# lfilipozzi/PathPlanning

Hardware: AMD Instinct MI355X
Metric: hybrid_astar_plans_per_sec_1024x1024 (higher is better)
Workload: dtype f64

## Files before the change

### pathplanning_amd/csrc/pp_pipeline.hpp

```cpp
#pragma once

#include <chrono>
#include <cstring>
#include <deque>
#include <unordered_map>

namespace {

__global__ void __launch_bounds__(256) k_pipe_scatter(int n, const int32_t* __restrict__ slotList, const double* __restrict__ startsIn, const double* __restrict__ goalsIn,
	const uint64_t* __restrict__ seedsIn, double* __restrict__ starts, double* __restrict__ goals, uint64_t* __restrict__ seeds, MapView m, float urgentClearance, PipeCtl* ctl,
	unsigned long long* __restrict__ urgent, unsigned long long urgentMask, int* __restrict__ claimed)
{
	const int i = (int)(blockIdx.x * blockDim.x + threadIdx.x);
	bool isUrgent = false;
	uint32_t entry = 0;
	if (i < n) {
		entry = (uint32_t)slotList[i];
		const size_t s = (size_t)(entry & pph::kSlotMask);
		for (int k = 0; k < 3; k++) {
			starts[3 * s + k] = startsIn[3 * (size_t)i + k];
			goals[3 * s + k] = goalsIn[3 * (size_t)i + k];
		}
		seeds[s] = seedsIn[i];
		if (claimed) {
// ... 248 lines not shown
{
	pp_planner* pl = P->pl;
	PP_HIP_TRY(pipe_stage_ctl(P, &P->ctl->nSubmitted, P->nSubmitted));
	PP_HIP_TRY(hipEventRecord(P->evCtl, P->ctlStream));
	hipStream_t s = nullptr;
	for (int i = 0; i < kPipeSearchStreams && !s; i++) {
		const int k = (P->nextSearch + i) % kPipeSearchStreams;
		if (hipStreamQuery(P->searchStream[k]) == hipSuccess) {
			s = P->searchStream[k];
			P->nextSearch = (k + 1) % kPipeSearchStreams;
		}
	}
	if (!s) {
		P->lastLaunch = std::chrono::steady_clock::now();
		return PP_OK;
	}
	PP_HIP_TRY(hipStreamWaitEvent(s, P->evCtl, 0));
	pl->args.rowsWaves = P->waves;
	pl->args.m = pl->map->view();
	const pp_pipeline::Timed tm = timed_take(P, s, 1, 0);
	PP_HIP_TRY(pipe_dispatch_search(P, s, pl->args));
	timed_done(P, s, tm);
	P->lastLaunch = std::chrono::steady_clock::now();
	return PP_OK;
}

bool pipe_dead(const pp_pipeline* P)
{
	if (P->dead)
		set_error("the pipeline failed earlier and must be destroyed");
	return P->dead;
}
int pipe_check(const pp_pipeline* P)
{
	if (!P) {
		set_error("null pipeline");
		return PP_ERR_INVALID;
	}
	return pipe_dead(P) ? PP_ERR_HIP : PP_OK;
}


int pipe_resolve(const pp_pipeline* P, int n, const uint64_t* tickets, const char* verb, bool distinct, std::vector<int32_t>& slots)
{
	pph::TicketTable::Resolved r = P->tickets.resolve(n, tickets, verb, distinct);
	slots.swap(r.slots);
	if (r.error.empty())
		return PP_OK;
	set_error(r.error);
	return PP_ERR_INVALID;
}
int pipe_refuse(const pp_pipeline* P, uint64_t ticket, const char* verb)
{
	std::vector<int32_t> none;
	if (pipe_resolve(P, 1, &ticket, verb, false, none) == PP_OK)
		set_error("ticket " + std::to_string(ticket) + " is not a completed, held query");
	return PP_ERR_INVALID;
}

bool pipe_release(pp_pipeline* P, uint64_t ticket)
{
	P->postIndexOfTicket.erase(ticket);
	return P->tickets.release(ticket);
}

hipError_t pipe_grow(pp_pipeline* P, size_t& capacity, size_t wanted, std::initializer_list<std::pair<pph::DeviceMem*, size_t>> buffers)
{
	const bool idle = P->nSubmitted == P->doneHead;
	if (idle)
		P->heldParked.clear();
	if (capacity >= wanted)
		return hipSuccess;
	capacity = 0;
	for (const auto& [buffer, bytes] : buffers) {
		if (!idle && buffer->get())
			P->heldParked.emplace_back(std::move(*buffer));
		if (const hipError_t e = buffer->alloc(bytes))
			return e;
	}
	capacity = wanted;
	return hipSuccess;
}

template <typename Rec, typename Launch>
int pipe_run_held(pp_pipeline* P, const std::vector<int32_t>& slots, const ppd::MapView& view, int32_t* slotsDev, const Rec* outDev, std::vector<Rec>& host, Launch launch)
{
	const int n = (int)slots.size();
	SearchArgs args = P->pl->args;
	args.m = view;
	Footprint foot {};
	if (P->footprint)
		foot = P->footprint->fp;
	hipStream_t s = P->ctlStream;
	PP_HIP_TRY(hipMemcpyAsync(slotsDev, slots.data(), (size_t)n * 4, hipMemcpyHostToDevice, s));
	launch(args, foot, n, (const int32_t*)slotsDev);
	PP_HIP_TRY(hipGetLastError());
	host.resize((size_t)n);
	PP_HIP_TRY(hipMemcpyAsync(host.data(), outDev, (size_t)n * sizeof(Rec), hipMemcpyDeviceToHost, s));
	PP_HIP_TRY(hipStreamSynchronize(s));
	return PP_OK;
}

}

extern "C" {

int pp_pipeline_create(pp_map* map, const pp_hybrid_params* params, int32_t capacity, int32_t max_nodes_per_query, int32_t search_rows, int32_t log_expansions, pp_pipeline** out)
{
	if (!map || !params || !out || capacity < 4 || capacity > (int32_t)pph::kSlotMask || max_nodes_per_query < 16 || search_rows < 0) {
		set_error("invalid arguments (4 <= capacity < 2^20)");
		return PP_ERR_INVALID;
	}
	PP_HIP_TRY(hipSetDevice(map->ctx->device));
	auto* P = new pp_pipeline();
	P->capacity = capacity;
	if (search_rows == 0)
		search_rows = 4096;
	if (int rc = create_planner(map, params, capacity, max_nodes_per_query, search_rows, log_expansions ? PlannerUse::PipelineLogged : PlannerUse::Pipeline, &P->pl)) {
		free_pipeline(P);
		return rc;
	}
	pp_planner* pl = P->pl;
	P->waves = pl->searchRows / kRowsPerWave;
	size_t ring = 4;
	while (ring < (size_t)capacity * 2)
		ring <<= 1;
	P->readyMask = P->doneMask = ring - 1;
	P->slotListCap = (size_t)capacity * 4;
	hipError_t e = hipSuccess;
#define PIPE_TRY(expr)         \
	do {                       \
		if (e == hipSuccess)   \
			e = (expr);        \
	} while (0)
	PIPE_TRY(P->ctl.alloc(sizeof(PipeCtl)));
	PIPE_TRY(P->ready.alloc(ring * 8));
	PIPE_TRY(P->waveAlive.alloc((size_t)P->waves * 4));
	PIPE_TRY(P->slotLists.alloc(P->slotListCap * 4));
	PIPE_TRY(P->urgent.alloc(ring * 8));
	PIPE_TRY(P->claimed.alloc((size_t)capacity * 4));
	if (const char* v = getenv("PP_PIPE_URGENT_CLEARANCE")) {
		const double x = strtod(v, nullptr);
		if (x >= 0.0 && x < 1.0e6)
			P->urgentClearance = (float)x;
	}
	if (const char* v = getenv("PP_PIPE_WF_STREAMS")) {
		const long x = strtol(v, nullptr, 10);
		if (x >= 1 && x <= kPipeWavefrontStreams)
			P->nWf = (int)x;
	}
	for (int i = 0; i < P->nWf; i++) {
		PIPE_TRY(P->wfWorkspace[i].alloc((size_t)pl->wfBytesPerSlot * pl->wfSlots));
		if (const size_t qw = pph::wavefront_tiles_queue_words(pl->map->desc.rows, pl->map->desc.cols)) {
			P->tilesQueueWaves = 2048;
			PIPE_TRY(P->tilesQueue[i].alloc(qw * 4 * (size_t)P->tilesQueueWaves));
		}
		PIPE_TRY(P->wfCtl[i].alloc(64));
		PIPE_TRY(hipMemset(P->wfCtl[i], 0, 64));
		PIPE_TRY(P->wfStream[i].create());
	}
	for (int i = 0; i < pp_pipeline::kFbSets; i++) {
		PIPE_TRY(P->fbCtl[i].alloc(64));
		PIPE_TRY(hipMemset(P->fbCtl[i], 0, 64));
		PIPE_TRY(P->fbList[i].alloc((size_t)capacity * 4));
		PIPE_TRY(P->fbDone[i].create(hipEventDisableTiming));
		PIPE_TRY(P->fbAfterTiles[i].create(hipEventDisableTiming));
	}
	PIPE_TRY(P->fbStream.create());
	int prioLow = 0, prioHigh = 0;
	(void)hipDeviceGetStreamPriorityRange(&prioLow, &prioHigh);
	const bool flatPriority = prioHigh == prioLow;
	if (flatPriority)
		prioHigh = 0;
	for (int i = 0; i < kPipeSearchStreams; i++)
		PIPE_TRY(P->searchStream[i].create(prioHigh));
	PIPE_TRY(P->ctlStream.create(prioHigh));
	PIPE_TRY(P->evIngest.create(hipEventDisableTiming));
	PIPE_TRY(P->evCtl.create(hipEventDisableTiming));
	PIPE_TRY(P->done.alloc(ring * sizeof(PipeDone)));
	PIPE_TRY(P->slotStage.alloc(P->slotListCap * 4));
	PIPE_TRY(P->submittedStage.alloc(64 * 8));
	PIPE_TRY(P->errFlags.alloc(64));
	if (const char* v = getenv("PP_PIPE_PATH_POSES")) {
		const long x = strtol(v, nullptr, 10);
		if (x >= 0 && x <= 2048)
			P->pathHostCap = (int)x;
	}
	if (P->pathHostCap > pl->maxPath)
		P->pathHostCap = pl->maxPath;
	if (P->pathHostCap > 0)
		PIPE_TRY(P->pathHost.alloc((size_t)capacity * (size_t)P->pathHostCap * 24));
	PIPE_TRY(hipMemset(P->ctl, 0, sizeof(PipeCtl)));
	PIPE_TRY(hipMemset(P->ready, 0, ring * 8));
	PIPE_TRY(hipMemset(P->waveAlive, 0, (size_t)P->waves * 4));
	PIPE_TRY(hipMemset(P->urgent, 0, ring * 8));
	PIPE_TRY(hipMemset(P->claimed, 0, (size_t)capacity * 4));
	PIPE_TRY(hipDeviceSynchronize());
#undef PIPE_TRY
	if (e != hipSuccess) {
		free_pipeline(P);
		return pph::hip_fail(e, "pipeline allocation");
	}
	{
		std::vector<hipStream_t> all;
		for (int i = 0; i < P->nWf; i++)
			all.push_back(P->wfStream[i]);
		for (hipStream_t st : P->searchStream)
			all.push_back(st);
		all.push_back(P->fbStream);
		const size_t nLong = all.size();
		all.push_back(P->ctlStream);
		pph::Dev<unsigned int> probeMem;
		e = probeMem.alloc(16);
		unsigned int* const probe = probeMem;
		for (size_t j = 0; j < all.size() && e == hipSuccess; j++)
			hipLaunchKernelGGL(k_queue_probe_set, dim3(1), dim3(64), 0, all[j], probe, 1u << j);
		if (e == hipSuccess)
			e = hipDeviceSynchronize();
		int seen[2] = { 1, 1 };
		int blockedBy = -1;
		unsigned int blockedMask = 0;
		for (size_t x = 0; x < nLong && e == hipSuccess && seen[1]; x++) {
			e = hipMemset(probe, 0, 16);
			if (e == hipSuccess)
				e = hipDeviceSynchronize();
			const bool xHigh = !flatPriority && x >= (size_t)P->nWf && x < (size_t)P->nWf + kPipeSearchStreams;
			unsigned int want = 0;
			for (size_t j = 0; j < all.size(); j++) {
				const bool jHigh = !flatPriority && ((j >= (size_t)P->nWf && j < (size_t)P->nWf + kPipeSearchStreams) || j + 1 == all.size());
				if (j != x && (!xHigh || jHigh))
					want |= 1u << j;
			}
			hipLaunchKernelGGL(k_queue_probe_hog, dim3(16384), dim3(64), 0, all[x], probe, want, reinterpret_cast<unsigned long long*>(probe + 2));
			for (size_t j = 0; j < all.size(); j++)
				if (j != x)
					hipLaunchKernelGGL(k_queue_probe_set, dim3(1), dim3(64), 0, all[j], probe, 1u << j);
			if (e == hipSuccess)
				e = hipDeviceSynchronize();
			unsigned int flags[2] = { 0, 0 };
			if (e == hipSuccess)
				e = hipMemcpy(flags, probe, 8, hipMemcpyDeviceToHost);
			seen[1] = flags[1] == 0 ? 1 : 0;
			if (!seen[1]) {
				blockedBy = (int)x;
				blockedMask = flags[1] & 0x7FFFFFFFu;
			}
		}
		if (e != hipSuccess) {
			free_pipeline(P);
			return pph::hip_fail(e, "pipeline queue probe");
		}
		const char* allow = getenv("PP_PIPE_ALLOW_SHARED_QUEUES");
		if (!seen[1] && !(allow && allow[0] == '1')) {
			free_pipeline(P);
			set_error("the pipeline's " + std::to_string(all.size()) + " streams do not run side by side (a launch waiting for room on stream " + std::to_string(blockedBy) +
				" holds back streams 0x" + [&] { char b[16]; snprintf(b, sizeof b, "%x", blockedMask); return std::string(b); }() +
				"; streams: wavefront, 4 x search, hand-over, control): the HIP runtime maps streams onto GPU_MAX_HW_QUEUES hardware "
				"queues (default 4, fixed when the runtime starts) and a wavefront launch queued behind the persistent search grid would wait for the grid's idle "
				"time-out.  Give the runtime a hardware queue per stream (GPU_MAX_HW_QUEUES in the environment before the process's first HIP call), or set "
				"PP_PIPE_ALLOW_SHARED_QUEUES=1 to run anyway (bench.py and the tests do)");
			return PP_ERR_INVALID;
		}
	}
	auto warmUp = [&](const char* what, auto&& launchEmpty) -> int {
		launchEmpty();
		e = hipGetLastError();
		if (e == hipSuccess)
			e = hipStreamSynchronize(P->ctlStream);
		if (e == hipSuccess)
			return PP_OK;
		free_pipeline(P);
		return pph::hip_fail(e, what);
	};
	if (int rc = warmUp("pipeline post-processing kernel warm-up (scratch allocation)", [&] {
			hipLaunchKernelGGL(k_postprocess_tickets, dim3(1), dim3(kPostThreads), 64, P->ctlStream, pl->args, PostParams {}, Footprint {}, 0, (const int32_t*)nullptr,
				(const PathRec*)nullptr, (const RsLogEntry*)nullptr, (const DevResult*)nullptr, (const uint32_t*)nullptr, (const uint32_t*)nullptr, PostBuffers {});
		}))
		return rc;
	if (int rc = warmUp("pipeline re-validation kernel warm-up (scratch allocation)", [&] {
			hipLaunchKernelGGL(k_revalidate_tickets, dim3(1), dim3(64), 0, P->ctlStream, pl->args, Footprint {}, 0, (const int32_t*)nullptr, (const PathRec*)nullptr,
				(const RsLogEntry*)nullptr, (const DevResult*)nullptr, (pp_revalidate_result*)nullptr);
		}))
		return rc;
	if (int rc = warmUp("pipeline stamp kernel warm-up (scratch allocation)", [&] {
			(void)launch_stamp(P->ctlStream, pl->args, Footprint {}, nullptr, 0, nullptr, nullptr, pl, nullptr, nullptr);
		}))
		return rc;
	std::memset(P->done, 0, ring * sizeof(PipeDone));
	std::memset(P->errFlags, 0, 64);
	P->tickets.reset(capacity);
	pl->hostResults.resize((size_t)capacity);
	pl->lastBatch = capacity;
	pl->pipelineOwned = true;
	pl->owner = P;
	{
		P->wfBlocks = pl->wfSlots;
		if (const char* b = getenv("PP_PIPE_WF_BLOCKS")) {
			const long x = strtol(b, nullptr, 10);
			if (x >= 1 && x < P->wfBlocks)
				P->wfBlocks = (int)x;
		}
		const char* v = getenv("PP_PIPE_IDLE_MS");
		if (v && *v) {
			const long ms = strtol(v, nullptr, 10);
			P->idleTicks = (unsigned long long)(ms < 1 ? 1 : (ms > 10000 ? 10000 : ms)) * 250ull;
		}
		P->lingerTicks = P->idleTicks;
// ... 630 lines not shown
```

### pathplanning_amd/csrc/pp_wavefront_tiles.hip

```cpp
#include <cstdio>
#include "pp_internal.hpp"

#include <cstdlib>
#include <type_traits>

using namespace ppd;

namespace {

constexpr int TT = 64;
template <int TW>
struct TileShape {
	static constexpr int LS = TW + 2;
	static constexpr int LN = (TT + 2) * LS;
	static constexpr int LNP = (LN + 3) & ~3;
	typedef typename std::conditional<TW == 64, uint64_t, uint32_t>::type Mask;
};
constexpr uint32_t kInfBits = 0x7F800000u;
#ifndef PP_WF_TILES_PRIO_DEFAULT
#define PP_WF_TILES_PRIO_DEFAULT 1
#endif
#ifndef PP_WF_TILE_WIDTH_DEFAULT
#define PP_WF_TILE_WIDTH_DEFAULT 32
#endif

__device__ __forceinline__ void wave_sync()
{
	__builtin_amdgcn_fence(__ATOMIC_ACQ_REL, "wavefront");
	__builtin_amdgcn_wave_barrier();
}
__device__ __forceinline__ uint32_t from_prev_lane(uint32_t v, uint32_t first) { return (uint32_t)__builtin_amdgcn_update_dpp((int)first, (int)v, 0x138, 0xF, 0xF, false); }
__device__ __forceinline__ uint32_t from_next_lane(uint32_t v, uint32_t last) { return (uint32_t)__builtin_amdgcn_update_dpp((int)last, (int)v, 0x130, 0xF, 0xF, false); }
__device__ __forceinline__ uint64_t from_prev_lane64(uint64_t v, uint64_t first)
{
	return (uint64_t)from_prev_lane((uint32_t)v, (uint32_t)first) | ((uint64_t)from_prev_lane((uint32_t)(v >> 32), (uint32_t)(first >> 32)) << 32);
}
__device__ __forceinline__ uint64_t from_next_lane64(uint64_t v, uint64_t last)
{
	return (uint64_t)from_next_lane((uint32_t)v, (uint32_t)last) | ((uint64_t)from_next_lane((uint32_t)(v >> 32), (uint32_t)(last >> 32)) << 32);
}
__device__ __forceinline__ uint32_t mask_from_prev(uint32_t v, uint32_t first) { return from_prev_lane(v, first); }
__device__ __forceinline__ uint32_t mask_from_next(uint32_t v, uint32_t last) { return from_next_lane(v, last); }
__device__ __forceinline__ uint64_t mask_from_prev(uint64_t v, uint64_t first) { return from_prev_lane64(v, first); }
__device__ __forceinline__ uint64_t mask_from_next(uint64_t v, uint64_t last) { return from_next_lane64(v, last); }
__device__ __forceinline__ uint32_t wave_min_u32(uint32_t v)
{
	const int id = (int)0xFFFFFFFF;
	uint32_t x = v;
	x = min(x, (uint32_t)__builtin_amdgcn_update_dpp(id, (int)x, 0x111, 0xF, 0xF, false));
	x = min(x, (uint32_t)__builtin_amdgcn_update_dpp(id, (int)x, 0x112, 0xF, 0xF, false));
	x = min(x, (uint32_t)__builtin_amdgcn_update_dpp(id, (int)x, 0x114, 0xF, 0xF, false));
	x = min(x, (uint32_t)__builtin_amdgcn_update_dpp(id, (int)x, 0x118, 0xF, 0xF, false));
	x = min(x, (uint32_t)__builtin_amdgcn_update_dpp(id, (int)x, 0x142, 0xA, 0xF, false));
	x = min(x, (uint32_t)__builtin_amdgcn_update_dpp(id, (int)x, 0x143, 0xC, 0xF, false));
	return (uint32_t)__builtin_amdgcn_readlane((int)x, 63);
}
__device__ __forceinline__ float wave_min_nonneg(float v) { return __uint_as_float(wave_min_u32(__float_as_uint(v))); }

template <int TW>
__device__ __forceinline__ void tile_cell(int tiledOut, int e, int& i, int& j)
{
	if (tiledOut) {
		const int ft = e >> (2 * kFieldTileLog2), within = e & ((1 << (2 * kFieldTileLog2)) - 1);
		constexpr int perRow = TW >> kFieldTileLog2;
		i = ((ft / perRow) << kFieldTileLog2) + (within >> kFieldTileLog2);
		j = ((ft % perRow) << kFieldTileLog2) + (within & kFieldTileMask);
	} else {
		i = e / TW;
		j = e % TW;
	}
}

__global__ void __launch_bounds__(256) k_occ_bits(const uint8_t* __restrict__ occ8, int rows, int cols, int wpr, int nWordRows, uint64_t* __restrict__ bits)
{
	const int64_t w = (int64_t)blockIdx.x * 4 + (threadIdx.x >> 6);
	const int lane = threadIdx.x & 63;
	if (w >= (int64_t)nWordRows * wpr)
		return;
	const int pr = (int)(w / wpr), pw = (int)(w - (int64_t)pr * wpr);
	const int r = pr - 1, c = (pw - 1) * 64 + lane;
	bool o = true;
	if (r >= 0 && r < rows && pw >= 1 && c < cols)
		o = occ8[(int64_t)r * cols + c] != 0;
	const uint64_t b = __ballot(o);
	if (lane == 0)
		bits[w] = b;
}

__global__ void __launch_bounds__(256) k_clearance_views(const float* __restrict__ dist, const uint8_t* __restrict__ occ8, int rows, int cols, int wpr, int nWordRows,
	float radius, uint8_t* __restrict__ blocked8, uint64_t* __restrict__ bits)
{
	const int64_t w = (int64_t)blockIdx.x * 4 + (threadIdx.x >> 6);
	const int lane = threadIdx.x & 63;
	if (w >= (int64_t)nWordRows * wpr)
		return;
	const int pr = (int)(w / wpr), pw = (int)(w - (int64_t)pr * wpr);
	const int r = pr - 1, c = (pw - 1) * 64 + lane;
	bool o = true;
	if (r >= 0 && r < rows && pw >= 1 && c < cols) {
		const int64_t cell = (int64_t)r * cols + c;
		o = occ8[cell] != 0 || !(dist[cell] >= radius);
		blocked8[cell] = o ? 1 : 0;
	}
	const uint64_t b = __ballot(o);
	if (lane == 0)
		bits[w] = b;
}

struct TilesArgs {
	MapView m;
	int nGoals;
	const int32_t* goalCells;
	const double* goalPoses;
	float* costOut;
	int tiledOut;
	int* ctl;
	int32_t* fbList;
	const double* orderStarts;
	float* orderKeys;
	unsigned long long* stats;
	int forceFallbackEvery;
	int ldsPerWave;
	int prio;
	pph::WavefrontPublish pub;
};

template <int TW, bool kProf, bool kGQ>
__global__ void __launch_bounds__(512) k_wavefront_tiles(TilesArgs A)
{
	unsigned long long ph[5] = { 0, 0, 0, 0, 0 }, tl = 0;
#define TILE_STAMP(i)                                        \
	if (kProf) {                                             \
		const unsigned long long now_ = __builtin_readcyclecounter(); \
		ph[i] += now_ - tl;                                  \
		tl = now_;                                           \
	}
	typedef typename TileShape<TW>::Mask Mask;
	constexpr int LS = TileShape<TW>::LS, LNP = TileShape<TW>::LNP;
	constexpr Mask kAll = (Mask)~(Mask)0;
	extern __shared__ __attribute__((aligned(16))) uint32_t smemAll[];
	const int lane = threadIdx.x & 63;
	uint32_t* const smemRaw = smemAll + (size_t)__builtin_amdgcn_readfirstlane((int)(threadIdx.x >> 6)) * (size_t)(A.ldsPerWave >> 2);
	if (A.prio == 1)
		__builtin_amdgcn_s_setprio(1);
	else if (A.prio == 2)
		__builtin_amdgcn_s_setprio(2);
	else if (A.prio == 3)
		__builtin_amdgcn_s_setprio(3);
	const MapView& m = A.m;
	const int rows = m.rows, cols = m.cols;
	const int TR = (rows + TT - 1) / TT, TC = (cols + TW - 1) / TW, nTiles = TR * TC;
	float* const L = reinterpret_cast<float*>(smemRaw);
	const uint32_t* const Lu = smemRaw;
	uint16_t* const tqL = reinterpret_cast<uint16_t*>(L + LNP);
	const int nTileWords = (nTiles + 1) >> 1;
	uint32_t* const tqG = kGQ ? A.pub.tilesQueue + ((size_t)blockIdx.x * (blockDim.x >> 6) + (threadIdx.x >> 6)) * (size_t)nTileWords : nullptr;
	constexpr uint32_t kNotQueued = 0x7FFFu;
	auto tq_word = [&](int w) -> uint32_t {
		if (kGQ)
			return __hip_atomic_load(tqG + w, __ATOMIC_RELAXED, __HIP_MEMORY_SCOPE_AGENT);
		return reinterpret_cast<const uint32_t*>(tqL)[w];
	};
	auto tq_get = [&](int t) -> uint32_t {
		if (kGQ)
			return (uint32_t)__hip_atomic_load(reinterpret_cast<uint16_t*>(tqG) + t, __ATOMIC_RELAXED, __HIP_MEMORY_SCOPE_AGENT);
		return (uint32_t)tqL[t];
	};
	auto tq_set = [&](int t, uint32_t v) {
		if (kGQ)
			__hip_atomic_store(reinterpret_cast<uint16_t*>(tqG) + t, (uint16_t)v, __ATOMIC_RELAXED, __HIP_MEMORY_SCOPE_AGENT);
		else
			tqL[t] = (uint16_t)v;
	};
	auto tq_sync = [&]() {
		if (kGQ)
			asm volatile("s_waitcnt vmcnt(0)" ::: "memory");
		else
			wave_sync();
	};
	const float kInf = __builtin_huge_valf();
	const float kDiag = sqrtf(2.0f);
	const int64_t cells = (int64_t)rows * cols;
	const int64_t fieldElems = A.tiledOut ? (int64_t)field_tiled_elems(rows, cols) : cells;
	const uint64_t* const occW = A.pub.occBits;
	const int wpr = (cols + 63) / 64 + 2;
	auto out_index = [&](int r, int c) -> size_t { return A.tiledOut ? field_tiled_index(cols, r, c) : (size_t)r * cols + c; };

	int pendingSlot = -1;
	bool ringTurn = true;
	unsigned long long stVisits = 0, stRounds = 0, stPasses = 0, stCells = 0, stGoals = 0, stFb = 0;
	const unsigned long long t0 = A.stats ? __builtin_readcyclecounter() : 0ull;
	for (;;) {
		asm volatile("s_waitcnt vmcnt(0)" ::: "memory");
		int next = -1, st = -1;
		if (lane == 0) {
			if (pendingSlot >= 0) {
				__builtin_amdgcn_fence(__ATOMIC_RELEASE, "agent");
				asm volatile("s_waitcnt vmcnt(0)" ::: "memory");
				const unsigned long long t = __hip_atomic_fetch_add(A.pub.readyTail, 1ull, __ATOMIC_RELAXED, __HIP_MEMORY_SCOPE_AGENT);
				__hip_atomic_store(A.pub.ready + (t & A.pub.readyMask), ((t + 1ull) << 32) | (unsigned long long)(uint32_t)pendingSlot, __ATOMIC_RELAXED, __HIP_MEMORY_SCOPE_AGENT);
			}
			auto take_urgent = [&]() -> int {
				for (;;) {
					unsigned long long h = __hip_atomic_load(A.pub.urgentHead, __ATOMIC_RELAXED, __HIP_MEMORY_SCOPE_AGENT);
					const unsigned long long e = __hip_atomic_load(A.pub.urgent + (h & A.pub.urgentMask), __ATOMIC_RELAXED, __HIP_MEMORY_SCOPE_AGENT);
					if ((uint32_t)(e >> 32) != (uint32_t)(h + 1ull))
						return -1;
					if (!__hip_atomic_compare_exchange_strong(A.pub.urgentHead, &h, h + 1ull, __ATOMIC_RELAXED, __ATOMIC_RELAXED, __HIP_MEMORY_SCOPE_AGENT))
						continue;
					const int slot = (int)((uint32_t)e & pph::kSlotMask);
					int expect = (int)(((uint32_t)e >> pph::kSlotBits) << 1);
					if (__hip_atomic_compare_exchange_strong(A.pub.claimed + slot, &expect, expect | 1, __ATOMIC_RELAXED, __ATOMIC_RELAXED, __HIP_MEMORY_SCOPE_AGENT))
						return slot;
				}
			};
			if (A.pub.urgent && ringTurn)
				next = take_urgent();
			while (next < 0) {
				const int gi = atomicAdd(A.ctl, 1);
				if (gi >= A.nGoals)
					break;
				if (!A.pub.slotList) {
					next = gi;
				} else {
					const uint32_t e = (uint32_t)A.pub.slotList[gi];
					const int slot = (int)(e & pph::kSlotMask);
					int expect = (int)((e >> pph::kSlotBits) << 1);
					if (!A.pub.claimed || __hip_atomic_compare_exchange_strong(A.pub.claimed + slot, &expect, expect | 1, __ATOMIC_RELAXED, __ATOMIC_RELAXED, __HIP_MEMORY_SCOPE_AGENT))
						next = slot;
				}
			}
			ringTurn = !ringTurn;
			if (next >= 0) {
				if (A.goalPoses) {
					double px, py;
					if (A.pub.claimed) {
						px = __hip_atomic_load(A.goalPoses + 3 * (size_t)next, __ATOMIC_RELAXED, __HIP_MEMORY_SCOPE_AGENT);
						py = __hip_atomic_load(A.goalPoses + 3 * (size_t)next + 1, __ATOMIC_RELAXED, __HIP_MEMORY_SCOPE_AGENT);
					} else {
						px = A.goalPoses[3 * (size_t)next];
						py = A.goalPoses[3 * (size_t)next + 1];
					}
					int row, col;
					world_to_cell(m, px, py, row, col);
					st = inside_map(m, row, col) ? row * m.cols + col : -1;
				} else {
					st = A.goalCells[next];
				}
			}
		}
		const int g = __builtin_amdgcn_readfirstlane(next);
		const int start = __builtin_amdgcn_readfirstlane(st);
		pendingSlot = -1;
		if (g < 0)
			break;
		if (kProf)
			stGoals++;
		float* const cost = A.costOut + (int64_t)g * fieldElems;
		const int goalR = start >= 0 ? start / cols : -1, goalC = start >= 0 ? start - goalR * cols : -1;

		if (kGQ) {
			for (int w = lane; w < nTileWords; w += 64)
				__hip_atomic_store(tqG + w, kNotQueued | (kNotQueued << 16), __ATOMIC_RELAXED, __HIP_MEMORY_SCOPE_AGENT);
		} else {
			for (int t = lane; t < ((nTiles + 1) & ~1); t += 64)
				tqL[t] = (uint16_t)kNotQueued;
		}
		tq_sync();
		if (start >= 0 && lane == 0)
			tq_set((goalR / TT) * TC + goalC / TW, 0u);
		tq_sync();
		bool flagged = false;
		int visits = 0;
		const int visitBudget = 6 * nTiles + 64;

		for (;;) {
			uint32_t bestBits = kNotQueued;
			int bestT = -1;
			if (kGQ)
				asm volatile("s_waitcnt vmcnt(0)" ::: "memory");
			for (int t2 = lane; t2 < (nTiles + 1) / 2; t2 += 64) {
				const uint32_t w = tq_word(t2);
				const uint32_t lo = w & 0x7FFFu, hi = (w >> 16) & 0x7FFFu;
				if (lo < bestBits) {
					bestBits = lo;
					bestT = 2 * t2;
				}
				if (hi < bestBits) {
					bestBits = hi;
					bestT = 2 * t2 + 1;
				}
			}
			const uint32_t minBits = wave_min_u32(bestBits);
			if (minBits == kNotQueued)
				break;
			const uint64_t who = __ballot(bestBits == minBits);
			const int t = __builtin_amdgcn_readlane(bestT, (int)__builtin_ctzll(who));
			if (++visits > visitBudget) {
				flagged = true;
				break;
			}
			if (kProf)
				tl = __builtin_readcyclecounter();
			const int tr = t / TC, tc = t - tr * TC;
			const int r0 = tr * TT, c0 = tc * TW;
			auto solved = [&](int dtr, int dtc) -> bool {
				const int a = tr + dtr, b = tc + dtc;
				return a >= 0 && b >= 0 && a < TR && b < TC && (tq_get(a * TC + b) & 0x8000u);
			};
			const bool selfSolved = solved(0, 0);
			asm volatile("s_waitcnt vmcnt(0)" ::: "memory");
			auto occ_bits = [&](int prow, int cFirst) -> Mask {
				const uint64_t w = occW[(size_t)prow * wpr + (size_t)((cFirst >> 6) + 1)];
				return (Mask)(w >> (cFirst & 63));
			};
			auto occ_bit = [&](int prow, int c) -> uint32_t {
				return (uint32_t)(occW[(size_t)prow * wpr + (size_t)((c >> 6) + 1)] >> (c & 63)) & 1u;
			};
			const Mask occ = occ_bits(r0 + lane + 1, c0);
			const uint32_t occL = occ_bit(r0 + lane + 1, c0 - 1), occR = occ_bit(r0 + lane + 1, c0 + TW);
			const Mask tH = occ_bits(r0, c0), bH = occ_bits(r0 + TT + 1, c0);
			const uint32_t tHL = occ_bit(r0, c0 - 1), tHR = occ_bit(r0, c0 + TW);
			const uint32_t bHL = occ_bit(r0 + TT + 1, c0 - 1), bHR = occ_bit(r0 + TT + 1, c0 + TW);
			float hT = kInf, hB = kInf, hL = kInf, hR = kInf, hC = kInf;
			float oT = kInf, oB = kInf, oL = kInf, oR = kInf;
			{
				const int cj = c0 + lane, ri = r0 + lane;
				if (lane < TW && cj < cols) {
					if (solved(-1, 0))
						hT = cost[out_index(r0 - 1, cj)];
					if (r0 + TT < rows && solved(1, 0))
						hB = cost[out_index(r0 + TT, cj)];
				}
				if (ri < rows) {
					if (solved(0, -1))
						hL = cost[out_index(ri, c0 - 1)];
					if (c0 + TW < cols && solved(0, 1))
						hR = cost[out_index(ri, c0 + TW)];
				}
				if (lane < 4) {
					const int dr = lane < 2 ? -1 : 1, dc = (lane & 1) ? 1 : -1;
					const int rr = dr < 0 ? r0 - 1 : r0 + TT, cc = dc < 0 ? c0 - 1 : c0 + TW;
					if (rr >= 0 && rr < rows && cc >= 0 && cc < cols && solved(dr, dc))
						hC = cost[out_index(rr, cc)];
				}
				if (selfSolved) {
					if (lane < TW && cj < cols) {
						oT = cost[out_index(r0, cj)];
						if (r0 + TT - 1 < rows)
							oB = cost[out_index(r0 + TT - 1, cj)];
					}
					if (ri < rows) {
						oL = cost[out_index(ri, c0)];
						if (c0 + TW - 1 < cols)
							oR = cost[out_index(ri, c0 + TW - 1)];
					}
				}
			}
			{
				float4* const L4 = reinterpret_cast<float4*>(L);
				const float4 inf4 = make_float4(kInf, kInf, kInf, kInf);
				for (int i = lane; i < LNP / 4; i += 64)
					L4[i] = inf4;
			}
			wave_sync();
			if (lane < TW) {
				L[lane + 1] = hT;
				L[(TT + 1) * LS + lane + 1] = hB;
			}
			L[(lane + 1) * LS] = hL;
			L[(lane + 1) * LS + TW + 1] = hR;
			if (lane < 4)
				L[(lane < 2 ? 0 : (TT + 1) * LS) + ((lane & 1) ? TW + 1 : 0)] = hC;
			Mask closed = occ, cur = 0, nx1 = 0, nx2 = 0;
			const bool goalHere = goalR >= r0 && goalR < r0 + TT && goalC >= c0 && goalC < c0 + TW;
			if (goalHere && lane == goalR - r0) {
				L[(lane + 1) * LS + (goalC - c0) + 1] = 0.0f;
				closed |= (Mask)1 << (goalC - c0);
				cur = (Mask)1 << (goalC - c0);
			}
			wave_sync();
			const int hbT = hT < kInf ? (int)hT : -1, hbB = hB < kInf ? (int)hB : -1, hbL = hL < kInf ? (int)hL : -1, hbR = hR < kInf ? (int)hR : -1, hbC = hC < kInf ? (int)hC : -1;
			int kmin;
			{
				uint32_t a = 0xFFFFFFFFu;
				a = min(a, (uint32_t)hbT);
				a = min(a, (uint32_t)hbB);
				a = min(a, (uint32_t)hbL);
				a = min(a, (uint32_t)hbR);
				a = min(a, (uint32_t)hbC);
				a = wave_min_u32(a);
				kmin = goalHere ? 0 : (int)a;
			}
			if (kProf)
				stVisits++;
			TILE_STAMP(0)
			if (kmin >= 0) {
				const Mask occUp = mask_from_prev(occ, tH), occDn = mask_from_next(occ, bH);
				const Mask occWst = (Mask)(occ << 1) | (Mask)occL, occEst = (Mask)(occ >> 1) | ((Mask)occR << (TW - 1));
				const Mask bNW = occUp & occWst, bNE = occUp & occEst, bSW = occDn & occWst, bSE = occDn & occEst;
				const Mask aNW = ~bNW, aNE = ~bNE, aSW = ~bSW, aSE = ~bSE;
				int k = kmin;
				for (;;) {
					const Mask topM = (Mask)__ballot(hbT == k), botM = (Mask)__ballot(hbB == k);
					const uint32_t cm = (uint32_t)__ballot(hbC == k) & 0xFu;
					const uint32_t lr = (hbL == k ? 1u : 0u) | (hbR == k ? 2u : 0u);
					const uint32_t lrU = from_prev_lane(lr, cm & 3u), lrD = from_next_lane(lr, (cm >> 2) & 3u);
					const Mask up = mask_from_prev(cur, topM), dn = mask_from_next(cur, botM);
					const Mask mW = (Mask)(cur << 1) | (Mask)(lr & 1u), mE = (Mask)(cur >> 1) | ((Mask)(lr >> 1) << (TW - 1));
					const Mask mNW = ((Mask)(up << 1) | (Mask)(lrU & 1u)) & aNW, mNE = ((Mask)(up >> 1) | ((Mask)(lrU >> 1) << (TW - 1))) & aNE;
					const Mask mSW = ((Mask)(dn << 1) | (Mask)(lrD & 1u)) & aSW, mSE = ((Mask)(dn >> 1) | ((Mask)(lrD >> 1) << (TW - 1))) & aSE;
					Mask cand = (mW | mE | up | dn | mNW | mNE | mSW | mSE) & (Mask)~closed;
					if (kProf)
						stRounds++;
					TILE_STAMP(1)
					const float kNext2 = (float)(k + 2);
					auto settle = [&](int j, uint32_t w, uint32_t e, uint32_t n, uint32_t s, uint32_t nw, uint32_t ne, uint32_t sw, uint32_t se) -> float {
						const uint32_t minS = min(min(w, e), min(n, s));
						auto blocked = [&](Mask b) -> uint32_t {
							if constexpr (sizeof(Mask) == 4)
								return (uint32_t)__builtin_amdgcn_sbfe((int)b, (unsigned)j, 1u);
							else
								return (uint32_t)-(int32_t)((uint32_t)(b >> j) & 1u);
						};
						uint32_t minD = nw | blocked(bNW);
						minD = min(minD, ne | blocked(bNE));
						minD = min(minD, sw | blocked(bSW));
						minD = min(minD, se | blocked(bSE));
						flagged |= minS == minD;
						return minS <= minD ? __uint_as_float(minS) + 1.0f : __uint_as_float(minD) + kDiag;
					};
					while (__ballot(cand != 0)) {
						if (kProf)
							stPasses++;
						if (cand != 0) {
							const int j0 = (int)__builtin_ctzll((uint64_t)cand);
							const Mask bit0 = (Mask)1 << j0;
							cand &= (Mask)~bit0;
							const bool two = cand != 0;
							const int j1 = two ? (int)__builtin_ctzll((uint64_t)cand) : j0;
							const Mask bit1 = (Mask)1 << j1;
							cand &= (Mask)~bit1;
							const int a0 = (lane + 1) * LS + j0 + 1, a1 = (lane + 1) * LS + j1 + 1;
							const uint32_t w0 = Lu[a0 - 1], e0 = Lu[a0 + 1], n0 = Lu[a0 - LS], s0 = Lu[a0 + LS];
							const uint32_t nw0 = Lu[a0 - LS - 1], ne0 = Lu[a0 - LS + 1], sw0 = Lu[a0 + LS - 1], se0 = Lu[a0 + LS + 1];
							const uint32_t w1 = Lu[a1 - 1], e1 = Lu[a1 + 1], n1 = Lu[a1 - LS], s1 = Lu[a1 + LS];
							const uint32_t nw1 = Lu[a1 - LS - 1], ne1 = Lu[a1 - LS + 1], sw1 = Lu[a1 + LS - 1], se1 = Lu[a1 + LS + 1];
							const float v0 = settle(j0, w0, e0, n0, s0, nw0, ne0, sw0, se0);
							const float v1 = settle(j1, w1, e1, n1, s1, nw1, ne1, sw1, se1);
							L[a0] = v0;
							if (two)
								L[a1] = v1;
							closed |= bit0 | bit1;
							nx1 |= (v0 < kNext2 ? bit0 : (Mask)0) | (v1 < kNext2 ? bit1 : (Mask)0);
							nx2 |= (v0 < kNext2 ? (Mask)0 : bit0) | (v1 < kNext2 ? (Mask)0 : bit1);
							if (kProf)
								stCells += two ? 2 : 1;
						}
						wave_sync();
					}
					TILE_STAMP(2)
					cur = nx1;
					nx1 = nx2;
					nx2 = 0;
					if (__ballot(closed != kAll) == 0ull)
						break;
					if (__ballot((cur | nx1) != 0) != 0ull) {
						k++;
					} else {
						uint32_t nb = 0xFFFFFFFFu;
						nb = min(nb, hbT > k ? (uint32_t)hbT : 0xFFFFFFFFu);
						nb = min(nb, hbB > k ? (uint32_t)hbB : 0xFFFFFFFFu);
						nb = min(nb, hbL > k ? (uint32_t)hbL : 0xFFFFFFFFu);
						nb = min(nb, hbR > k ? (uint32_t)hbR : 0xFFFFFFFFu);
						nb = min(nb, hbC > k ? (uint32_t)hbC : 0xFFFFFFFFu);
						nb = wave_min_u32(nb);
						if (nb == 0xFFFFFFFFu)
							break;
						k = (int)nb;
					}
				}
			}
			wave_sync();
			{
				const int lc = lane < TW ? lane : 0;
				const float nT = lane < TW ? L[LS + lc + 1] : kInf, nB = lane < TW ? L[TT * LS + lc + 1] : kInf, nL = L[(lane + 1) * LS + 1], nR = L[(lane + 1) * LS + TW];
				auto sees = [&](float p, float q, uint32_t qOcc) -> bool { return !qOcc && (q == kInf || p < q - 0.99f); };
				const uint32_t occLU = from_prev_lane(occL, tHL), occLD = from_next_lane(occL, bHL);
				const uint32_t occRU = from_prev_lane(occR, tHR), occRD = from_next_lane(occR, bHR);
				float pN = kInf, pS = kInf, pW = kInf, pE = kInf, pNW = kInf, pNE = kInf, pSW = kInf, pSE = kInf;
				{
					const bool ch = lane < TW && __float_as_uint(nT) != __float_as_uint(oT);
					const float p = fminf(nT, oT);
					const uint32_t o0 = lc == 0 ? tHL : (uint32_t)(tH >> (lc - 1)) & 1u, o1 = (uint32_t)(tH >> lc) & 1u, o2 = lc == TW - 1 ? tHR : (uint32_t)(tH >> (lc + 1)) & 1u;
					const bool c0_ = ch && sees(p, L[lc], o0), c1_ = ch && sees(p, L[lc + 1], o1), c2_ = ch && sees(p, L[lc + 2], o2);
					if (c1_ || (lc > 0 && c0_) || (lc < TW - 1 && c2_))
						pN = p;
					if (lc == 0 && c0_)
						pNW = p;
					if (lc == TW - 1 && c2_)
						pNE = p;
				}
				{
					const bool ch = lane < TW && __float_as_uint(nB) != __float_as_uint(oB);
					const float p = fminf(nB, oB);
					const float* const Lb = L + (TT + 1) * LS;
					const uint32_t o0 = lc == 0 ? bHL : (uint32_t)(bH >> (lc - 1)) & 1u, o1 = (uint32_t)(bH >> lc) & 1u, o2 = lc == TW - 1 ? bHR : (uint32_t)(bH >> (lc + 1)) & 1u;
					const bool c0_ = ch && sees(p, Lb[lc], o0), c1_ = ch && sees(p, Lb[lc + 1], o1), c2_ = ch && sees(p, Lb[lc + 2], o2);
					if (c1_ || (lc > 0 && c0_) || (lc < TW - 1 && c2_))
						pS = p;
					if (lc == 0 && c0_)
						pSW = p;
					if (lc == TW - 1 && c2_)
						pSE = p;
				}
				{
					const bool ch = __float_as_uint(nL) != __float_as_uint(oL);
					const float p = fminf(nL, oL);
					const bool c0_ = ch && sees(p, L[lane * LS], occLU), c1_ = ch && sees(p, L[(lane + 1) * LS], occL), c2_ = ch && sees(p, L[(lane + 2) * LS], occLD);
					if (c1_ || (lane > 0 && c0_) || (lane < 63 && c2_))
						pW = p;
					if (lane == 0 && c0_)
						pNW = fminf(pNW, p);
					if (lane == 63 && c2_)
						pSW = fminf(pSW, p);
				}
				{
					const bool ch = __float_as_uint(nR) != __float_as_uint(oR);
					const float p = fminf(nR, oR);
					const bool c0_ = ch && sees(p, L[lane * LS + TW + 1], occRU), c1_ = ch && sees(p, L[(lane + 1) * LS + TW + 1], occR), c2_ = ch && sees(p, L[(lane + 2) * LS + TW + 1], occRD);
					if (c1_ || (lane > 0 && c0_) || (lane < 63 && c2_))
						pE = p;
					if (lane == 0 && c0_)
						pNE = fminf(pNE, p);
					if (lane == 63 && c2_)
						pSE = fminf(pSE, p);
				}
				const float qN = wave_min_nonneg(pN), qS = wave_min_nonneg(pS), qW = wave_min_nonneg(pW), qE = wave_min_nonneg(pE);
				const float qNW = wave_min_nonneg(pNW), qNE = wave_min_nonneg(pNE), qSW = wave_min_nonneg(pSW), qSE = wave_min_nonneg(pSE);
				if (lane < 9) {
					const int dtr = lane < 2 ? (lane == 0 ? -1 : 1) : (lane < 4 ? 0 : (lane < 6 ? -1 : (lane < 8 ? 1 : 0)));
					const int dtc = lane < 2 ? 0 : (lane < 4 ? (lane == 2 ? -1 : 1) : (lane < 8 ? ((lane & 1) ? 1 : -1) : 0));
					const float p = lane == 0 ? qN : lane == 1 ? qS : lane == 2 ? qW : lane == 3 ? qE : lane == 4 ? qNW : lane == 5 ? qNE : lane == 6 ? qSW : lane == 7 ? qSE : kInf;
					const int a = tr + dtr, b = tc + dtc;
					if (lane == 8) {
						tq_set(t, 0x8000u | kNotQueued);
					} else if (p < kInf && a >= 0 && b >= 0 && a < TR && b < TC) {
						const uint32_t bucket = p < 32766.0f ? (uint32_t)p : 32766u, old = tq_get(a * TC + b);
						if (bucket < (old & 0x7FFFu))
							tq_set(a * TC + b, (old & 0x8000u) | bucket);
					}
				}
			}
			TILE_STAMP(3)
			for (int u = 0; u < TW; u++) {
				int i, j;
				tile_cell<TW>(A.tiledOut, u * TT + lane, i, j);
				const int r = r0 + i, c = c0 + j;
				if (r < rows && c < cols)
					cost[out_index(r, c)] = L[(i + 1) * LS + j + 1];
			}
			wave_sync();
			TILE_STAMP(4)
		}
		flagged = __ballot(flagged) != 0ull;
		if (!flagged) {
			for (int t = 0; t < nTiles; t++) {
				if (tq_get(t) & 0x8000u)
					continue;
				const int tr = t / TC, tc = t - tr * TC;
				for (int u = 0; u < TW; u++) {
					int i, j;
					tile_cell<TW>(A.tiledOut, u * TT + lane, i, j);
					const int r = tr * TT + i, c = tc * TW + j;
					if (r < rows && c < cols)
						cost[out_index(r, c)] = kInf;
				}
			}
		}
		if (A.forceFallbackEvery > 0 && (g % A.forceFallbackEvery) == A.forceFallbackEvery - 1)
			flagged = true;
		if (flagged) {
			if (kProf)
				stFb++;
			if (lane == 0)
				A.fbList[atomicAdd(A.ctl + 2, 1)] = g;
			continue;
		}
		if (A.pub.ready)
			pendingSlot = g;
		if (A.orderKeys) {
			asm volatile("s_waitcnt vmcnt(0)" ::: "memory");
			if (lane == 0) {
				int row, col;
				world_to_cell(m, A.orderStarts[3 * (size_t)g], A.orderStarts[3 * (size_t)g + 1], row, col);
				float c = kInf;
				if (inside_map(m, row, col))
					c = cost[out_index(row, col)];
				__hip_atomic_store(A.orderKeys + g, c, __ATOMIC_RELAXED, __HIP_MEMORY_SCOPE_AGENT);
			}
		}
	}
	if (kProf && A.stats && lane == 0) {
		atomicAdd(A.stats + 0, stGoals);
		atomicAdd(A.stats + 1, stVisits);
		atomicAdd(A.stats + 2, stRounds);
		atomicAdd(A.stats + 3, stPasses);
		atomicAdd(A.stats + 5, stFb);
		atomicAdd(A.stats + 6, (unsigned long long)(__builtin_readcyclecounter() - t0));
		if (kProf)
			for (int i = 0; i < 5; i++)
				atomicAdd(A.stats + 8 + i, ph[i]);
	}
#undef TILE_STAMP
	if (kProf && A.stats)
		atomicAdd(A.stats + 4, stCells);
	if (lane == 0) {
		__builtin_amdgcn_fence(__ATOMIC_RELEASE, "agent");
		if (__hip_atomic_fetch_add(A.ctl + 1, 1, __ATOMIC_RELAXED, __HIP_MEMORY_SCOPE_AGENT) == (int)(gridDim.x * (blockDim.x >> 6)) - 1) {
			__hip_atomic_store(A.ctl, 0, __ATOMIC_RELAXED, __HIP_MEMORY_SCOPE_AGENT);
			__hip_atomic_store(A.ctl + 1, 0, __ATOMIC_RELAXED, __HIP_MEMORY_SCOPE_AGENT);
		}
	}
}

__global__ void __launch_bounds__(512) k_order_by_key(int n, const float* __restrict__ keys, int32_t* __restrict__ orderOut)
{
	__shared__ unsigned long long skey[4096];
	const int tid = threadIdx.x;
	int P = 1;
	while (P < n)
		P <<= 1;
	for (int i = tid; i < P; i += 512) {
		unsigned long long v = 0ull;
		if (i < n)
			v = ((unsigned long long)(__float_as_uint(keys[i]) + 1u) << 32) | (unsigned long long)(0xFFFFFFFFu - (uint32_t)i);
		skey[i] = v;
	}
	__syncthreads();
	for (int kk = 2; kk <= P; kk <<= 1)
		for (int j = kk >> 1, lj = 31 - __clz(kk >> 1); j > 0; j >>= 1, lj--) {
			for (int t = tid; t < P / 2; t += 512) {
				const int i1 = ((t >> lj) << (lj + 1)) | (t & (j - 1)), i2 = i1 + j;
				const bool desc = (i1 & kk) == 0;
				const unsigned long long a = skey[i1], b = skey[i2];
				if ((a < b) == desc) {
					skey[i1] = b;
					skey[i2] = a;
				}
			}
			__syncthreads();
		}
	for (int i = tid; i < n; i += 512)
		orderOut[i] = (int32_t)(0xFFFFFFFFu - (uint32_t)skey[i]);
}

int tile_width()
{
	static const int w = [] {
		const char* e = getenv("PP_WF_TILE_WIDTH");
		return e && atoi(e) == 64 ? 64 : (e && atoi(e) == 32 ? 32 : PP_WF_TILE_WIDTH_DEFAULT);
	}();
	return w;
}

size_t tiles_count(int rows, int cols)
{
	const int tw = tile_width();
	return (size_t)((rows + TT - 1) / TT) * (size_t)((cols + tw - 1) / tw);
}

size_t tiles_lds_bytes(int rows, int cols, bool queueInGlobal = false)
{
	const size_t nTiles = tiles_count(rows, cols);
	return ((size_t)(tile_width() == 64 ? TileShape<64>::LNP : TileShape<32>::LNP) * 4 + (queueInGlobal ? 0 : ((nTiles + 1) & ~(size_t)1) * 2) + 15) & ~(size_t)15;
}

int waves_per_pack(size_t ldsPerWave)
{
	static const int forced = [] {
		const char* e = getenv("PP_WF_TILES_PACK");
		return e ? atoi(e) : 0;
	}();
	if (forced >= 1 && forced <= 8)
		return forced;
	int n = (int)((80 * 1024) / ldsPerWave) + 1;
	while (n > 1 && (size_t)n * ldsPerWave > 160 * 1024)
		n--;
	return n > 8 ? 8 : n;
}

void launch_tiles_kernel(hipStream_t s, int waves, TilesArgs A)
{
	const bool gq = A.pub.tilesQueue && A.pub.tilesQueueWaves > 0 && !A.stats;
	const size_t lds = tiles_lds_bytes(A.m.rows, A.m.cols, gq);
	static const bool trace = getenv("PP_WF_TILES_TRACE") != nullptr;
	if (trace && A.nGoals > 0)
		fprintf(stderr, "[tiles] launch: %d waves, tile queue in %s\n", waves, gq ? "global memory" : "LDS");
	const int pack = A.pub.ready ? waves_per_pack(lds) : 1;
	static const size_t minPackLds = [] {
		const char* e = getenv("PP_WF_TILES_PACK_KB");
		const int v = e ? atoi(e) : 82;
		return (size_t)(v < 1 ? 1 : (v > 160 ? 160 : v)) * 1024;
	}();
	const size_t packLds = pack > 1 && (size_t)pack * lds < minPackLds ? minPackLds : (size_t)pack * lds;
	A.ldsPerWave = (int)lds;
	static const int prio = [] {
		const char* e = getenv("PP_WF_TILES_PRIO");
		const int v = e ? atoi(e) : PP_WF_TILES_PRIO_DEFAULT;
		return v < 0 ? 0 : (v > 3 ? 3 : v);
	}();
	A.prio = prio;
	if (gq && waves > A.pub.tilesQueueWaves / pack * pack)
		waves = A.pub.tilesQueueWaves / pack * pack;
	const int grid = (waves + pack - 1) / pack;
	static const bool attr = [] {
		(void)hipFuncSetAttribute(reinterpret_cast<const void*>(k_wavefront_tiles<64, false, false>), hipFuncAttributeMaxDynamicSharedMemorySize, 160 * 1024);
		(void)hipFuncSetAttribute(reinterpret_cast<const void*>(k_wavefront_tiles<32, false, false>), hipFuncAttributeMaxDynamicSharedMemorySize, 160 * 1024);
		(void)hipFuncSetAttribute(reinterpret_cast<const void*>(k_wavefront_tiles<64, true, false>), hipFuncAttributeMaxDynamicSharedMemorySize, 160 * 1024);
		(void)hipFuncSetAttribute(reinterpret_cast<const void*>(k_wavefront_tiles<32, true, false>), hipFuncAttributeMaxDynamicSharedMemorySize, 160 * 1024);
		(void)hipFuncSetAttribute(reinterpret_cast<const void*>(k_wavefront_tiles<64, false, true>), hipFuncAttributeMaxDynamicSharedMemorySize, 160 * 1024);
		(void)hipFuncSetAttribute(reinterpret_cast<const void*>(k_wavefront_tiles<32, false, true>), hipFuncAttributeMaxDynamicSharedMemorySize, 160 * 1024);
		return true;
	}();
	(void)attr;
	if (tile_width() == 64) {
		if (A.stats)
			hipLaunchKernelGGL((k_wavefront_tiles<64, true, false>), dim3(grid), dim3(64 * pack), packLds, s, A);
		else if (gq)
			hipLaunchKernelGGL((k_wavefront_tiles<64, false, true>), dim3(grid), dim3(64 * pack), packLds, s, A);
		else
			hipLaunchKernelGGL((k_wavefront_tiles<64, false, false>), dim3(grid), dim3(64 * pack), packLds, s, A);
	} else {
		if (A.stats)
			hipLaunchKernelGGL((k_wavefront_tiles<32, true, false>), dim3(grid), dim3(64 * pack), packLds, s, A);
		else if (gq)
			hipLaunchKernelGGL((k_wavefront_tiles<32, false, true>), dim3(grid), dim3(64 * pack), packLds, s, A);
		else
			hipLaunchKernelGGL((k_wavefront_tiles<32, false, false>), dim3(grid), dim3(64 * pack), packLds, s, A);
	}
}

}

namespace pph {

void occ_bits_dims(int rows, int cols, int& wpr, int& nWordRows)
{
	wpr = (cols + TT - 1) / TT + 2;
	nWordRows = (rows + TT - 1) / TT * TT + 2;
}

hipError_t launch_occ_bits(hipStream_t s, const uint8_t* occ8, int rows, int cols, uint64_t* bits)
{
	int wpr, nWordRows;
	occ_bits_dims(rows, cols, wpr, nWordRows);
	const int64_t words = (int64_t)wpr * nWordRows;
	hipLaunchKernelGGL(k_occ_bits, dim3((unsigned)((words + 3) / 4)), dim3(256), 0, s, occ8, rows, cols, wpr, nWordRows, bits);
	return hipGetLastError();
}

hipError_t launch_clearance_views(hipStream_t s, const float* dist, const uint8_t* occ8, int rows, int cols, float radius, uint8_t* blocked8, uint64_t* bits)
{
	int wpr, nWordRows;
	occ_bits_dims(rows, cols, wpr, nWordRows);
	const int64_t words = (int64_t)wpr * nWordRows;
	hipLaunchKernelGGL(k_clearance_views, dim3((unsigned)((words + 3) / 4)), dim3(256), 0, s, dist, occ8, rows, cols, wpr, nWordRows, radius, blocked8, bits);
	return hipGetLastError();
}

bool wavefront_tiles_supported(int rows, int cols)
{
	return tiles_lds_bytes(rows, cols) <= 64 * 1024;
}

size_t wavefront_tiles_queue_words(int rows, int cols)
{
	static const bool global = [] {
		const char* e = getenv("PP_WF_TILES_QUEUE");
		return e && e[0] == 'g';
	}();
	return global ? (tiles_count(rows, cols) + 1) / 2 : 0;
}

int wavefront_tiles_resident_blocks(int rows, int cols)
{
	int perCu = 0, dev = 0;
	hipDeviceProp_t prop;
	if (hipGetDevice(&dev) != hipSuccess || hipGetDeviceProperties(&prop, dev) != hipSuccess)
		return 1024;
	const size_t lds = tiles_lds_bytes(rows, cols);
	const int pack = 1;
	const hipError_t e = tile_width() == 64 ? hipOccupancyMaxActiveBlocksPerMultiprocessor(&perCu, k_wavefront_tiles<64, false, false>, 64 * pack, lds * pack)
	                                        : hipOccupancyMaxActiveBlocksPerMultiprocessor(&perCu, k_wavefront_tiles<32, false, false>, 64 * pack, lds * pack);
	if (e != hipSuccess || perCu < 1)
		perCu = 1;
	return perCu * pack * prop.multiProcessorCount;
}

hipError_t warm_up_wavefront_tiles(hipStream_t s, const MapView& m, int* ctlDev)
{
	TilesArgs A {};
	A.m = m;
	A.ctl = ctlDev;
	launch_tiles_kernel(s, 1, A);
	return hipGetLastError();
}

hipError_t launch_wavefront_tiles(hipStream_t s, const MapView& m, const WavefrontLaunch& L)
{
	const WavefrontPublish& pub = L.pub;
	const int nGoals = L.nGoals;
	TilesArgs A {};
	A.m = m;
	A.nGoals = nGoals;
	A.goalCells = L.goalCells;
	A.goalPoses = L.goalPoses;
	A.costOut = L.cost;
	A.tiledOut = L.tiledOut ? 1 : 0;
	A.ctl = pub.tilesCtl;
	A.fbList = pub.tilesFallback;
	A.orderStarts = L.orderStarts;
	A.orderKeys = L.orderStarts ? L.orderKeys : nullptr;
	A.stats = pub.tilesStats;
	A.pub = pub;
	static const int forceEvery = [] {
		const char* e = getenv("PP_WF_TILES_FORCE_FALLBACK");
		return e ? atoi(e) : 0;
	}();
	A.forceFallbackEvery = forceEvery;
	static int resident = 0;
	static int residentRows = 0, residentCols = 0;
	if (!resident || residentRows != m.rows || residentCols != m.cols) {
		resident = wavefront_tiles_resident_blocks(m.rows, m.cols);
		residentRows = m.rows;
		residentCols = m.cols;
	}
	int grid = nGoals < resident ? nGoals : resident;
	if (const char* e = getenv("PP_WF_TILES_GRID")) {
		const int g = atoi(e);
		if (g > 0 && g < grid)
			grid = g;
	}
	launch_tiles_kernel(s, grid, A);
	return hipGetLastError();
}

hipError_t launch_order_by_key(hipStream_t s, int n, const float* keysDev, int32_t* orderOutDev)
{
	hipLaunchKernelGGL(k_order_by_key, dim3(1), dim3(512), 0, s, n, keysDev, orderOutDev);
	return hipGetLastError();
}
// ... 3 lines not shown
```

Before: 38450.

## Retune tile-kernel occupancy, pack sizing and lane register pressure

```diff
diff --git a/pathplanning_amd/csrc/pp_pipeline.hpp b/pathplanning_amd/csrc/pp_pipeline.hpp
--- a/pathplanning_amd/csrc/pp_pipeline.hpp
+++ b/pathplanning_amd/csrc/pp_pipeline.hpp
@@ -424,7 +424,7 @@
 	for (int i = 0; i < P->nWf; i++) {
 		PIPE_TRY(P->wfWorkspace[i].alloc((size_t)pl->wfBytesPerSlot * pl->wfSlots));
 		if (const size_t qw = pph::wavefront_tiles_queue_words(pl->map->desc.rows, pl->map->desc.cols)) {
-			P->tilesQueueWaves = 2048;
+			P->tilesQueueWaves = 2560;
 			PIPE_TRY(P->tilesQueue[i].alloc(qw * 4 * (size_t)P->tilesQueueWaves));
 		}
 		PIPE_TRY(P->wfCtl[i].alloc(64));
diff --git a/pathplanning_amd/csrc/pp_wavefront_tiles.hip b/pathplanning_amd/csrc/pp_wavefront_tiles.hip
--- a/pathplanning_amd/csrc/pp_wavefront_tiles.hip
+++ b/pathplanning_amd/csrc/pp_wavefront_tiles.hip
@@ -17,9 +17,14 @@
 	typedef typename std::conditional<TW == 64, uint64_t, uint32_t>::type Mask;
 };
 constexpr uint32_t kInfBits = 0x7F800000u;
+constexpr int kMaxPack = 10;
 #ifndef PP_WF_TILES_PRIO_DEFAULT
 #define PP_WF_TILES_PRIO_DEFAULT 1
 #endif
+#ifndef PP_WF_TILES_PACK_MAX_DEFAULT
+#define PP_WF_TILES_PACK_MAX_DEFAULT 8
+#endif
+static_assert(PP_WF_TILES_PACK_MAX_DEFAULT >= 1 && PP_WF_TILES_PACK_MAX_DEFAULT <= kMaxPack, "a pack's waves: 1..kMaxPack");
 #ifndef PP_WF_TILE_WIDTH_DEFAULT
 #define PP_WF_TILE_WIDTH_DEFAULT 32
 #endif
@@ -54,6 +59,11 @@
 	x = min(x, (uint32_t)__builtin_amdgcn_update_dpp(id, (int)x, 0x142, 0xA, 0xF, false));
 	x = min(x, (uint32_t)__builtin_amdgcn_update_dpp(id, (int)x, 0x143, 0xC, 0xF, false));
 	return (uint32_t)__builtin_amdgcn_readlane((int)x, 63);
+}
+__device__ __forceinline__ int recompute_from(int v)
+{
+	asm volatile("" : "+v"(v));
+	return v;
 }
 __device__ __forceinline__ float wave_min_nonneg(float v) { return __uint_as_float(wave_min_u32(__float_as_uint(v))); }
 
@@ -126,7 +136,7 @@
 };
 
 template <int TW, bool kProf, bool kGQ>
-__global__ void __launch_bounds__(512) k_wavefront_tiles(TilesArgs A)
+__global__ void __launch_bounds__(64 * kMaxPack) __attribute__((amdgpu_waves_per_eu(TW == 32 ? 6 : 1, TW == 32 ? 6 : 8))) k_wavefront_tiles(TilesArgs A)
 {
 	unsigned long long ph[5] = { 0, 0, 0, 0, 0 }, tl = 0;
 #define TILE_STAMP(i)                                        \
@@ -139,7 +149,8 @@
 	constexpr int LS = TileShape<TW>::LS, LNP = TileShape<TW>::LNP;
 	constexpr Mask kAll = (Mask)~(Mask)0;
 	extern __shared__ __attribute__((aligned(16))) uint32_t smemAll[];
-	const int lane = threadIdx.x & 63;
+	const int laneOfWave = threadIdx.x & 63;
+	const int lane = laneOfWave;
 	uint32_t* const smemRaw = smemAll + (size_t)__builtin_amdgcn_readfirstlane((int)(threadIdx.x >> 6)) * (size_t)(A.ldsPerWave >> 2);
 	if (A.prio == 1)
 		__builtin_amdgcn_s_setprio(1);
@@ -230,7 +241,6 @@
 						next = slot;
 				}
 			}
-			ringTurn = !ringTurn;
 			if (next >= 0) {
 				if (A.goalPoses) {
 					double px, py;
@@ -249,6 +259,7 @@
 				}
 			}
 		}
+		ringTurn = !ringTurn;
 		const int g = __builtin_amdgcn_readfirstlane(next);
 		const int start = __builtin_amdgcn_readfirstlane(st);
 		pendingSlot = -1;
@@ -304,6 +315,7 @@
 				tl = __builtin_readcyclecounter();
 			const int tr = t / TC, tc = t - tr * TC;
 			const int r0 = tr * TT, c0 = tc * TW;
+			const int lane = recompute_from(laneOfWave);
 			auto solved = [&](int dtr, int dtc) -> bool {
 				const int a = tr + dtr, b = tc + dtc;
 				return a >= 0 && b >= 0 && a < TR && b < TC && (tq_get(a * TC + b) & 0x8000u);
@@ -431,8 +443,10 @@
 						return minS <= minD ? __uint_as_float(minS) + 1.0f : __uint_as_float(minD) + kDiag;
 					};
 					while (__ballot(cand != 0)) {
-						if (kProf)
+						if (kProf) {
 							stPasses++;
+							stCells += __popcll(__ballot(cand != 0)) + __popcll(__ballot((cand & (cand - 1)) != 0));
+						}
 						if (cand != 0) {
 							const int j0 = (int)__builtin_ctzll((uint64_t)cand);
 							const Mask bit0 = (Mask)1 << j0;
@@ -454,8 +468,6 @@
 							closed |= bit0 | bit1;
 							nx1 |= (v0 < kNext2 ? bit0 : (Mask)0) | (v1 < kNext2 ? bit1 : (Mask)0);
 							nx2 |= (v0 < kNext2 ? (Mask)0 : bit0) | (v1 < kNext2 ? (Mask)0 : bit1);
-							if (kProf)
-								stCells += two ? 2 : 1;
 						}
 						wave_sync();
 					}
@@ -483,6 +495,7 @@
 			}
 			wave_sync();
 			{
+				const int lane = recompute_from(laneOfWave);
 				const int lc = lane < TW ? lane : 0;
 				const float nT = lane < TW ? L[LS + lc + 1] : kInf, nB = lane < TW ? L[TT * LS + lc + 1] : kInf, nL = L[(lane + 1) * LS + 1], nR = L[(lane + 1) * LS + TW];
 				auto sees = [&](float p, float q, uint32_t qOcc) -> bool { return !qOcc && (q == kInf || p < q - 0.99f); };
@@ -553,9 +566,10 @@
 				}
 			}
 			TILE_STAMP(3)
+			const int laneS = recompute_from(laneOfWave);
 			for (int u = 0; u < TW; u++) {
 				int i, j;
-				tile_cell<TW>(A.tiledOut, u * TT + lane, i, j);
+				tile_cell<TW>(A.tiledOut, u * TT + laneS, i, j);
 				const int r = r0 + i, c = c0 + j;
 				if (r < rows && c < cols)
 					cost[out_index(r, c)] = L[(i + 1) * LS + j + 1];
@@ -606,6 +620,7 @@
 		atomicAdd(A.stats + 1, stVisits);
 		atomicAdd(A.stats + 2, stRounds);
 		atomicAdd(A.stats + 3, stPasses);
+		atomicAdd(A.stats + 4, stCells);
 		atomicAdd(A.stats + 5, stFb);
 		atomicAdd(A.stats + 6, (unsigned long long)(__builtin_readcyclecounter() - t0));
 		if (kProf)
@@ -613,8 +628,6 @@
 				atomicAdd(A.stats + 8 + i, ph[i]);
 	}
 #undef TILE_STAMP
-	if (kProf && A.stats)
-		atomicAdd(A.stats + 4, stCells);
 	if (lane == 0) {
 		__builtin_amdgcn_fence(__ATOMIC_RELEASE, "agent");
 		if (__hip_atomic_fetch_add(A.ctl + 1, 1, __ATOMIC_RELAXED, __HIP_MEMORY_SCOPE_AGENT) == (int)(gridDim.x * (blockDim.x >> 6)) - 1) {
@@ -682,12 +695,14 @@
 		const char* e = getenv("PP_WF_TILES_PACK");
 		return e ? atoi(e) : 0;
 	}();
-	if (forced >= 1 && forced <= 8)
+	if (forced >= 1 && forced <= kMaxPack)
 		return forced;
-	int n = (int)((80 * 1024) / ldsPerWave) + 1;
-	while (n > 1 && (size_t)n * ldsPerWave > 160 * 1024)
+	constexpr size_t kCuLds = 160 * 1024, kSearchLdsPerCu = 4 * 14 * 1024;
+	const int half = (int)((kCuLds / 2) / ldsPerWave) + 1, beside = (int)((kCuLds - kSearchLdsPerCu) / ldsPerWave);
+	int n = half > beside ? half : beside;
+	while (n > 1 && (size_t)n * ldsPerWave > kCuLds)
 		n--;
-	return n > 8 ? 8 : n;
+	return n > PP_WF_TILES_PACK_MAX_DEFAULT ? PP_WF_TILES_PACK_MAX_DEFAULT : n;
 }
 
 void launch_tiles_kernel(hipStream_t s, int waves, TilesArgs A)
@@ -695,9 +710,9 @@
 	const bool gq = A.pub.tilesQueue && A.pub.tilesQueueWaves > 0 && !A.stats;
 	const size_t lds = tiles_lds_bytes(A.m.rows, A.m.cols, gq);
 	static const bool trace = getenv("PP_WF_TILES_TRACE") != nullptr;
+	const int pack = A.pub.ready ? waves_per_pack(lds) : 1;
 	if (trace && A.nGoals > 0)
-		fprintf(stderr, "[tiles] launch: %d waves, tile queue in %s\n", waves, gq ? "global memory" : "LDS");
-	const int pack = A.pub.ready ? waves_per_pack(lds) : 1;
+		fprintf(stderr, "[tiles] launch: %d waves in packs of %d, tile queue in %s\n", waves, pack, gq ? "global memory" : "LDS");
 	static const size_t minPackLds = [] {
 		const char* e = getenv("PP_WF_TILES_PACK_KB");
 		const int v = e ? atoi(e) : 82;
```

New measurement: 35330. 0.919x the previous value.
